# warmshao/ChatTTSPlus

Measured on AMD Instinct MI355X. Metric: decode tokens/s, higher is better.
Workload: dtype f32

## Files before the change

chatttsplus_amd/csrc/gpt_engine.hip:

```cpp
#include <fcntl.h>
#include <stdarg.h>
#include <stdio.h>
#include <stdlib.h>
#include <string.h>
#include <sys/file.h>
#include <sys/stat.h>
#include <unistd.h>

#include <cmath>
#include <map>
#include <mutex>
#include <string>
#include <atomic>
#include <thread>
#include <vector>

#include "../../include/ctts_hip.h"
#include "kernels.h"
#include "persist.h"
#include "roctx_range.h"

static thread_local char g_err[512] = "";
void ctts_set_error(const char* fmt, ...) {
    va_list ap;
// ... 1360 lines not shown
        CTTS_HIP_CHECK(hipMemcpyAsync(h->x_pre, emb + (size_t)r0 * h->H, (size_t)n * h->H * 4, hipMemcpyDeviceToDevice, s));
        if (run_layers(h, h->x_pre, h->meta_pre + r0, h->rope_pre + (size_t)r0 * 64, n, DecodePath{1, 0}, nullptr, s)) return 1;
        sr.cum[0] = 0;
        for (int b = 0; b < B; ++b) {
            const long s0 = (long)b * T + T - n_targets[b], s1 = (long)b * T + T;
            const long lo = s0 > r0 ? s0 : r0, hi = s1 < r0 + n ? s1 : r0 + n;
            const int cnt = hi > lo ? (int)(hi - lo) : 0;
            sr.first[b] = cnt ? (int)(lo - r0) : 0;
            sr.j0[b] = cnt ? (int)(lo - s0) : 0;
            sr.cum[b + 1] = sr.cum[b] + cnt;
        }
        for (int g0 = 0; g0 < sr.cum[B]; g0 += SCORE_ROWS) {
            const int m = sr.cum[B] - g0 < SCORE_ROWS ? sr.cum[B] - g0 : SCORE_ROWS;
            if (launch_score_gather(h->x_pre, h->score_x, h->score_oidx, g0, m, sr, s)) return 1;
            GemmArgs a = {};
            a.R = m; a.eps = 1e-6f; a.W = h->whead; a.n_row_tiles = (NV + 15) / 16; a.K = h->H; a.x = h->score_x; a.lnw = h->lnf;
            a.logits = h->score_logits; a.n_valid = NV;
            if (launch_gemm(h->cfg.dtype, nbg, PRO_NORM, EPI_LOGITS, a, (m + 16 * nbg - 1) / (16 * nbg), s)) return 1;
            if (launch_score_reduce(h->score_logits, h->score_oidx, targets, logprob, argmax, m, h->V, NV, s)) return 1;
        }
    }
    return 0;
}

static int run_decode_step(ctts_gpt* h, DecodePath path, hipStream_t s);
static inline DecodePath pick_decode_path(const ctts_gpt* h, int longest);

extern "C" int ctts_gpt_set_logprob_out(ctts_gpt* h, float* lp_raw, float* lp_sampled, void* stream) {
    if (!h || h->B == 0) { ctts_set_error("set_logprob_out: no generate state (call ctts_gpt_begin first)"); return 1; }
    if (h->text_mode) { ctts_set_error("set_logprob_out: the refine-text pass (infer_text) returns no log-probs; code mode only"); return 1; }
    if (h->sampled) { ctts_set_error("set_logprob_out: called after the first ctts_gpt_sample / ctts_gpt_decode of this call; set the buffers right after ctts_gpt_begin"); return 1; }
    float* const p[2] = {lp_raw, lp_sampled};
    static_assert(offsetof(SamplerDyn, lp_sampled) == offsetof(SamplerDyn, lp_raw) + sizeof(float*), "the two destinations are copied as one pair");
    CTTS_HIP_CHECK(hipMemcpyAsync((char*)h->dyn + offsetof(SamplerDyn, lp_raw), p, sizeof(p), hipMemcpyHostToDevice, (hipStream_t)stream));
    return 0;
}

extern "C" int ctts_gpt_sample(ctts_gpt* h, void* stream) {
    if (!h || h->B == 0) { ctts_set_error("sample: call begin first"); return 1; }
    CTTS_RANGE("ctts_gpt_sample");
    h->sampled = true;
    if (h->batch_inv) {
        if (ensure_persist_images(h)) return 1;
        return run_decode_step(h, pick_decode_path(h, 0), (hipStream_t)stream);
    }
    return run_sample_phase(h, plain_form(h), (hipStream_t)stream);
}

extern "C" int ctts_gpt_restart(ctts_gpt* h, void* stream) {
    if (!h || h->B == 0) { ctts_set_error("restart: call begin first"); return 1; }
    if (h->B != h->B0) { ctts_set_error("restart: rows were compacted away (a regenerate restarts the whole batch at step 0, gpt.py:496-525)"); return 1; }
    if (h->admitted) { ctts_set_error("restart: rows of this batch were handed to other utterances (ctts_gpt_admit); re-admit the utterance with attempt + 1 instead"); return 1; }
    hipStream_t s = (hipStream_t)stream;
    CTTS_HIP_CHECK(hipMemcpyAsync(h->x_dec, h->x_last, (size_t)h->B * h->H * 4, hipMemcpyDeviceToDevice, s));
    if (h->batch_inv) CTTS_HIP_CHECK(hipMemcpyAsync(h->rope_dec, h->rope_dec0, (size_t)h->B * 64 * 4, hipMemcpyDeviceToDevice, s));
    return reset_state(h, true, s);
}

static int advance_rows(ctts_gpt* h, int n_steps) {
    int longest = 1;
    for (int r = 0; r < h->B; ++r) {
        int c = h->row_ctx[r] + n_steps;
        if (c > h->row_cap[r]) c = h->row_cap[r];
        h->row_ctx[r] = c;
        if (c > longest) longest = c;
    }
    return longest;
}

static inline int decode_persist(const ctts_gpt* h, int B, int L) {
    const int rows = tuning(h).persist_rows;
    if (!(rows > 0 && h->pimg != nullptr && B <= rows && B <= PL_MAXR)) return 0;
    if (h->lora_rows && h->lora_mlp) return 0;
    if (h->lora_rows && !(h->persist_lora && h->persist_sched == 3 && h->lora_Af != nullptr && h->H == PL_H)) return 0;
    int cap = PL_ATT_BLOCKS / (PL_NH * B);
    cap = cap > PL_SMAX ? PL_SMAX : (cap < 1 ? 1 : cap);
    if (h->persist_splits > 0) cap = h->persist_splits < cap ? h->persist_splits : cap;
    if (B > PL_MAXR_ONE) {
        if (h->persist_sched != 3) return 0;
        return (L > (h->persist_max_keys > 0 ? h->persist_max_keys : h->persist_pair_keys - 128 * (B - PL_MAXR_ONE - 1))) ? 0 : 1;
    }
    if (L > (h->persist_max_keys > 0 ? h->persist_max_keys : 1400 * cap)) return 0;
    const int share = h->persist_share_keys > 0 ? h->persist_share_keys : PL_SHARE_KEYS;
    if (L <= share + 128) return 1;
    const int want = (L + share - 1) / share;
    return want > cap ? cap : want;
}

static inline DecodePath pick_decode_path(const ctts_gpt* h, int longest) { return {decode_splits(h, h->B, longest), decode_persist(h, h->B, longest)}; }

struct PersistTurn {
    std::mutex mu;
    hipEvent_t ev = nullptr;
    hipStream_t last = nullptr;
    bool pending = false;
};
static PersistTurn* persist_turn() {
    static std::mutex mu;
    static std::map<int, PersistTurn*> turns;
    int dev = 0;
    if (hipGetDevice(&dev) != hipSuccess) return nullptr;
    std::lock_guard<std::mutex> lk(mu);
    auto it = turns.find(dev);
    if (it != turns.end()) return it->second;
    PersistTurn* t = new PersistTurn();
    if (hipEventCreateWithFlags(&t->ev, hipEventDisableTiming) != hipSuccess) { delete t; return nullptr; }
    turns[dev] = t;
    return t;
}
struct PersistTurnGuard {
    PersistTurn* t = nullptr;
    hipStream_t s = nullptr;
    int rc = 0;
    PersistTurnGuard(bool persistent, hipStream_t stream) : s(stream) {
        if (!persistent) return;
        t = persist_turn();
        if (!t) return;
        t->mu.lock();
        if (t->pending && t->last != s && hipStreamWaitEvent(s, t->ev, 0) != hipSuccess) rc = 1;
    }
    ~PersistTurnGuard() {
        if (!t) return;
        if (hipEventRecord(t->ev, s) == hipSuccess) { t->last = s; t->pending = true; }
        t->mu.unlock();
    }
};

static int run_decode_step(ctts_gpt* h, DecodePath path, hipStream_t s) {
    StreamForm form = {};
    if (run_layers(h, h->x_dec, h->meta_dec, h->rope_dec, h->B, path, h->st, s, &form)) return 1;
    return run_sample_phase(h, form, s);
}

static int graph_span(const ctts_gpt* h, DecodePath path, int left) {
    return (path.persist && h->graph_steps_persist > h->graph_steps && left >= h->graph_steps_persist) ? h->graph_steps_persist : h->graph_steps;
}

static int ensure_graph(ctts_gpt* h, DecodePath path, int n_steps) {
    char sig[160];
    snprintf(sig, sizeof(sig), "%d|%d|%p|%d|%d|%d|%d|%d", h->B, h->text_mode, (void*)h->kv, path.splits, h->lora_rows + 2 * h->lora_mlp, h->opt_gen, path.persist, n_steps);
    std::string key(sig);
    if (h->lora_rows) key.append((const char*)h->lora_row_slots, (size_t)h->B);
    if (h->graph_gen != h->opt_gen || h->graphs.size() >= 96) {
        if (!h->graphs.empty()) {
            CTTS_HIP_CHECK(hipDeviceSynchronize());
            for (auto& kv : h->graphs) { (void)hipGraphExecDestroy(kv.second.exec); (void)hipGraphDestroy(kv.second.graph); }
            h->graphs.clear(); h->gexec = nullptr;
        }
        h->graph_gen = h->opt_gen;
    }
    auto it = h->graphs.find(key);
    if (it != h->graphs.end()) { h->gexec = it->second.exec; return 0; }
    ctts_gpt::GraphEntry ge = {nullptr, nullptr};
    CTTS_HIP_CHECK(hipStreamBeginCapture(h->cap_stream, hipStreamCaptureModeThreadLocal));
    int rc = 0;
    for (int i = 0; i < n_steps && !rc; ++i) rc = run_decode_step(h, path, h->cap_stream);
    hipError_t e = hipStreamEndCapture(h->cap_stream, &ge.graph);
    if (rc) { if (ge.graph) (void)hipGraphDestroy(ge.graph); return 1; }
    if (e != hipSuccess) { ctts_set_error("hipStreamEndCapture: %s", hipGetErrorString(e)); return 1; }
    e = hipGraphInstantiate(&ge.exec, ge.graph, nullptr, nullptr, 0);
    if (e != hipSuccess) { (void)hipGraphDestroy(ge.graph); ctts_set_error("hipGraphInstantiate: %s", hipGetErrorString(e)); return 1; }
    h->graphs[key] = ge;
    h->gexec = ge.exec;
    return 0;
}

static void plan_decode(ctts_gpt* h, int n_steps) {
// ... 311 lines not shown
```

chatttsplus_amd/csrc/persist.h:

```cpp
#pragma once
#include "common.h"

#define PL_GEMV_BLOCKS 192
#define PL_ATT_BLOCKS 64
#define PL_BLOCKS (PL_GEMV_BLOCKS + PL_ATT_BLOCKS)
#ifndef PL_EW_ONE_ROW
#define PL_EW_ONE_ROW 4
#endif
#define PL_EDGE_WAVES(R) ((R) == 1 ? PL_EW_ONE_ROW : 4)
#define PL_THREADS(R) ((8 + PL_EDGE_WAVES(R)) * 64)
#define PL_THREADS_MAX 768
#define PL_H 768
#define PL_I 3072
#define PL_NH 12
#define PL_MAXR_ONE 5
#define PL_MAXR 8
#define PL_SHARE_KEYS 384
#define PL_QKV_BYTES (12 * 768 * 4)
#define PL_O_BYTES (4 * 768 * 4)
#define PL_GU_BYTES (32 * 768 * 4)
#define PL_D_BYTES (4 * 3072 * 4)
#define PL_BLOCK_BYTES (PL_QKV_BYTES + PL_O_BYTES + PL_GU_BYTES + PL_D_BYTES)
#define PL_LAYER_BYTES ((size_t)PL_GEMV_BLOCKS * PL_BLOCK_BYTES)
#define PL_G_QKV (PL_MAXR * PL_NH * 192)
#define PL_G_ATT (PL_MAXR * PL_H)
#define PL_G_X1 (PL_MAXR * PL_H)
#define PL_G_ACT (PL_MAXR * PL_I)
#define PL_G_X (PL_MAXR * PL_H)
#define PL_SMAX 5
#define PL_G_PART (PL_ATT_BLOCKS * 66)
#define PL_HEAD_ROWS 14
#define PL_HEAD_FRAGS (7 * 2 * 3 * 64)
#define PL_G_U (PL_MAXR * 64)
#define PL_G_TOTAL (PL_G_QKV + PL_G_ATT + PL_G_X1 + PL_G_ACT + PL_G_X + PL_G_PART + PL_G_U)

struct PersistArgs {
    const char* w;
    const char* hw;
    int heads;
    float* logits;
    int n_valid;
    const float* lnf;
    const SamplerDyn* dyn;
    const RowState* rows;
    int half_w;
    int n_layers;
    float* x;
    const RowMeta* meta;
    const float* rope_rows;
    void* kv;
    size_t kv_per;
    int Lmax;
    unsigned long long* g_qkv;
    unsigned long long* g_att;
    unsigned long long* g_x1;
    unsigned long long* g_act;
    unsigned long long* g_x;
    unsigned long long* g_part;
    int S;
    unsigned* epoch;
    int* error;
    const int* done;
    unsigned long long* ts;
    float eps;
    int sched;
    int pace;
    int delay_act, delay_x, nap_qkv;
    int delay_att, delay;
    int nap;
    int fault;
    int poll;
    int lora;
    int delay_u;
    unsigned long long lslots;
    const float* la_qkv;
    const float* la;
    const float* lb;
    const float* lscale;
    size_t la_qkv_stride, la_stride;
    unsigned long long* g_u;
};

int launch_persist_layer(int R, const PersistArgs& a, hipStream_t s);
int launch_persist_repack_heads(int half_w, const void* whead, int n_tiles, void* dst, hipStream_t s);
int launch_persist_repack(int half_w, const void* qkv, const void* o, const void* gu, const void* d, void* dst, hipStream_t s);
int persist_configure();
```

chatttsplus_amd/csrc/persist_layer.hip:

```cpp
#include "kernels.h"
#include "persist.h"

typedef unsigned long long u64;

#ifndef PL_LB
#define PL_LB PL_THREADS_MAX
#endif
#define PL_SPIN_LIMIT (1u << 18)

typedef __attribute__((address_space(3))) int pl_lds_int;
#define PL_ABORT_GET(p_) __hip_atomic_load((pl_lds_int*)(p_), __ATOMIC_RELAXED, __HIP_MEMORY_SCOPE_WORKGROUP)
#define PL_ABORT_SET(p_) __hip_atomic_store((pl_lds_int*)(p_), 1, __ATOMIC_RELAXED, __HIP_MEMORY_SCOPE_WORKGROUP)
__device__ inline void store_granule(u64* g, unsigned tag, float v) {
    __hip_atomic_store(g, ((u64)tag << 32) | (u64)__builtin_bit_cast(unsigned, v), __ATOMIC_RELAXED, __HIP_MEMORY_SCOPE_AGENT);
}

template <int N, typename OffFn>
__device__ inline bool sweep(const u64* base, unsigned lane_elem, OffFn off, unsigned tag, float (&v)[N], int* err, int code, int* abort_s, int nap = 1) {
    const u64* p = base + lane_elem;
    asm volatile("" : "+v"(p));
#pragma unroll 1
    for (unsigned spins = 0;; ++spins) {
        bool ok = true;
#pragma unroll
// ... 66 lines not shown
    const __amdgpu_buffer_rsrc_t rsrc = __builtin_amdgcn_make_buffer_rsrc((void*)base, 0, (int)(total * 16u), 0x00020000);
    const unsigned voff = f0 * 16u;
#pragma unroll 1
    for (unsigned spins = 0;; ++spins) {
        bool ok = true;
#pragma unroll
        for (int k = 0; k < N; ++k) {
            const pl_u32x4 x = __builtin_amdgcn_raw_buffer_load_b128(rsrc, (int)voff, (int)(k * stride * 16u), (int)(16u | 0x80000000u));
            v[k] = x;
            if (TAIL && k == N - 1) ok = ok && ((x[3] - x[0] - x[1] - x[2] == tag) || (f0 + k * stride >= total));
            else ok = ok && (x[3] - x[0] - x[1] - x[2] == tag);
        }
        if (__all(ok)) return true;
        bool giveup = spins >= PL_SPIN_LIMIT || PL_ABORT_GET(abort_s) != 0;
        if (!giveup && (spins & 1023u) == 1023u) giveup = __hip_atomic_load(err, __ATOMIC_RELAXED, __HIP_MEMORY_SCOPE_AGENT) != 0;
        if (giveup) {
            if ((threadIdx.x & 63) == 0) { atomicCAS(err, 0, code); PL_ABORT_SET(abort_s); }
            return false;
        }
        for (int z = 0; z < nap; ++z) __builtin_amdgcn_s_sleep(2);
    }
}
template <int K0, int N, int NE, int TOT>
__device__ __forceinline__ void act16_chunk(const void* g_act, int e, unsigned tag, __attribute__((address_space(3))) float* xs, int* err, int* abort_s, int nap) {
    pl_u32x4 v[N];
    constexpr bool TAIL = (NE * (K0 + N) > TOT);
    const bool got = sweep16<N, TAIL>(g_act, (unsigned)TOT, (unsigned)(e + NE * K0), (unsigned)NE, tag, v, err, 5, abort_s, nap);
    (void)got;
    int ee = e;
    asm volatile("" : "+v"(ee));
#pragma unroll
    for (int k = 0; k < N; ++k) {
        const int f = ee + NE * (K0 + k);
        if (!(TAIL && k == N - 1) || f < TOT) {
            const int P = f / PL_A16_SLOTS, s = f - PL_A16_SLOTS * P;
            __attribute__((address_space(3))) float* const d = xs + 16 * P + 3 * s;
            const unsigned w0 = v[k][0], w1 = v[k][1], w2 = v[k][2];
            d[0] = __builtin_bit_cast(float, w0);
            if (s < 5) { d[1] = __builtin_bit_cast(float, w1); d[2] = __builtin_bit_cast(float, w2); }
        }
    }
}

template <typename OffFn>
__device__ inline void watch_sentinels(const u64* base, OffFn off, int n, unsigned tag, int lane, int* abort_s) {
    const u64* p0 = base + ((lane < n) ? off(lane) : 0);
    const u64* p1 = base + ((lane + 64 < n) ? off(lane + 64) : 0);
    asm volatile("" : "+v"(p0), "+v"(p1));
#pragma unroll 1
    for (unsigned spins = 0; spins < 8192u; ++spins) {
        bool ok = true;
        if (lane < n) ok = (unsigned)(__hip_atomic_load(p0, __ATOMIC_RELAXED, __HIP_MEMORY_SCOPE_AGENT) >> 32) == tag;
        if (lane + 64 < n) ok = ok && ((unsigned)(__hip_atomic_load(p1, __ATOMIC_RELAXED, __HIP_MEMORY_SCOPE_AGENT) >> 32) == tag);
        if (__all(ok) || PL_ABORT_GET(abort_s) != 0) return;
        __builtin_amdgcn_s_sleep(2);
    }
}

template <bool ON> __device__ inline int pl_opq(int idx) {
    if constexpr (ON) asm volatile("" : "+v"(idx));
    return idx;
}
__device__ inline float dot4(const f32x4 w, const f32x4 x, float acc) {
    return fmaf(w[3], x[3], fmaf(w[2], x[2], fmaf(w[1], x[1], fmaf(w[0], x[0], acc))));
}
__device__ inline float dot4(const half4 w, const f32x4 x, float acc) {
    return fmaf((float)w[3], x[3], fmaf((float)w[2], x[2], fmaf((float)w[1], x[1], fmaf((float)w[0], x[0], acc))));
}
template <typename WT> struct PlW;
template <> struct PlW<float> { typedef f32x4 frag; };
template <> struct PlW<half_t> { typedef half4 frag; };
template <typename WT> struct PlKV;
template <> struct PlKV<float> {
    f32x4 a, b;
    __device__ inline void load(const float* p) { a = *(const f32x4*)p; b = *(const f32x4*)(p + 4); }
    __device__ inline float at(int j) const { return j < 4 ? a[j & 3] : b[j & 3]; }
};
template <> struct PlKV<half_t> {
    half8 h;
    __device__ inline void load(const half_t* p) { h = *(const half8*)p; }
    __device__ inline float at(int j) const { return (float)h[j]; }
};
__device__ inline float pl_exp_diff(float m, float mn) { return (m == -INFINITY) ? 0.f : expf(m - mn); }

constexpr int pl_pow2(int n) { return n <= 1 ? 1 : n <= 2 ? 2 : n <= 4 ? 4 : n <= 8 ? 8 : 16; }
template <int CTRL, int C> __device__ inline void pl_rs_step(float* v, bool f) {
    if constexpr (C > 1) {
#pragma unroll
        for (int i = 0; i < C / 2; ++i) {
            const float keep = f ? v[i + C / 2] : v[i];
            const float give = f ? v[i] : v[i + C / 2];
            v[i] = keep + dpp_f<CTRL>(give);
        }
    } else v[0] += dpp_f<CTRL>(v[0]);
}
#define PL_FRONT_BYTES 4096
#ifndef PL_TAIL_ALL
#define PL_TAIL_ALL 1
#endif
#ifndef PL_TAIL_IT
#define PL_TAIL_IT 4
#endif
#define PL_RED_FLOATS (8 * 32 * 4)
template <int P> __device__ inline void pl_reduce_store(float (&v)[P], float* red, int wave, int lane, int base = 0) {
    static_assert(P == 1 || P == 2 || P == 4 || P == 8 || P == 16, "pad to a power of two");
    constexpr int C1 = P > 1 ? P / 2 : 1, C2 = P > 2 ? P / 4 : 1, C3 = P > 4 ? P / 8 : 1;
    const bool f0 = ((lane ^ (lane >> 2)) & 1) != 0, f1 = (((lane >> 1) ^ (lane >> 2)) & 1) != 0, f2 = (((lane >> 2) ^ (lane >> 3)) & 1) != 0, f3 = ((lane >> 3) & 1) != 0;
    pl_rs_step<DPP_XOR1, P>(v, f0);
    pl_rs_step<DPP_XOR2, C1>(v, f1);
    pl_rs_step<DPP_HALF_MIRROR, C2>(v, f2);
    pl_rs_step<DPP_MIRROR, C3>(v, f3);
    int idx = 0;
    bool writer = true;
    if (P > 1) idx += f0 ? P / 2 : 0; else writer = writer && !f0;
    if (C1 > 1) idx += f1 ? C1 / 2 : 0; else writer = writer && !f1;
    if (C2 > 1) idx += f2 ? C2 / 2 : 0; else writer = writer && !f2;
    if (C3 > 1) idx += f3 ? C3 / 2 : 0; else writer = writer && !f3;
    if (writer) red[(wave * 32 + base + idx) * 4 + (lane >> 4)] = v[0];
}
__device__ inline float pl_red(const float* red, int wave, int n) {
    const f32x4 p = *(const f32x4*)(red + (wave * 32 + n) * 4);
    return (p[0] + p[1]) + (p[2] + p[3]);
}
#define PL_PV(N_) float pv[pl_pow2(N_)]; _Pragma("unroll") for (int n_ = 0; n_ < pl_pow2(N_); ++n_) pv[n_] = 0.f

__device__ inline int pl_slot(unsigned long long slots, int r) { return (int)(signed char)(unsigned char)(slots >> (8 * r)); }
template <typename WT> struct PlLoraRegs {
    f32x4 qa_[3], qb_[3], oa_[3], ob_;
    template <typename Q> __device__ inline f32x4& qa(Q&, int j) { return qa_[j]; }
    template <typename Q> __device__ inline f32x4& qb(Q&, int j) { return qb_[j]; }
    template <typename O> __device__ inline f32x4& oa(O&, int j) { return oa_[j]; }
    template <typename Q> __device__ inline f32x4& ob(Q&) { return ob_; }
};
template <> struct PlLoraRegs<float> {
    __device__ inline f32x4& qa(f32x4 (&q_w)[2][3], int j) { return q_w[0][j]; }
    __device__ inline f32x4& qb(f32x4 (&q_w)[2][3], int j) { return q_w[1][j]; }
    __device__ inline f32x4& oa(f32x4 (&o_w)[3], int j) { return o_w[j]; }
    __device__ inline f32x4& ob(f32x4 (&q_w)[2][3]) { return q_w[0][0]; }
};
template <int N>
__device__ inline bool sweep_masked(const u64* base, unsigned lane_elem, bool valid, unsigned tag, float (&v)[N], int* err, int code, int* abort_s, int nap) {
    const u64* p = base + (valid ? lane_elem : 0u);
    asm volatile("" : "+v"(p));
#pragma unroll
    for (int k = 0; k < N; ++k) v[k] = 0.f;
    if (!__any(valid)) return true;
#pragma unroll 1
    for (unsigned spins = 0;; ++spins) {
        bool ok = true;
        if (valid) {
#pragma unroll
            for (int k = 0; k < N; ++k) {
                const u64 x = __hip_atomic_load(p + k, __ATOMIC_RELAXED, __HIP_MEMORY_SCOPE_AGENT);
                v[k] = __builtin_bit_cast(float, (unsigned)x);
                ok = ok && ((unsigned)(x >> 32) == tag);
            }
        }
        if (__all(ok)) return true;
        bool giveup = spins >= PL_SPIN_LIMIT || PL_ABORT_GET(abort_s) != 0;
        if (!giveup && (spins & 1023u) == 1023u) giveup = __hip_atomic_load(err, __ATOMIC_RELAXED, __HIP_MEMORY_SCOPE_AGENT) != 0;
        if (giveup) {
            if ((threadIdx.x & 63) == 0) { atomicCAS(err, 0, code); PL_ABORT_SET(abort_s); }
            return false;
        }
        for (int z = 0; z < nap; ++z) __builtin_amdgcn_s_sleep(2);
    }
}

template <int R, int SCHED, typename WT, bool LORA = false>
__global__ __launch_bounds__(PL_LB) void persist_layer_kernel(const PersistArgs a) {
    static_assert(!LORA || SCHED == 3, "per-utterance adapters: the paced schedule only");
    typedef typename PlW<WT>::frag wfrag;
    constexpr bool A16 = PL_ACT16 != 0 && R <= PL_A16_MAXR;
    constexpr int EW = PL_EDGE_WAVES(R), NE = 64 * EW, GX = 768 / NE;
    constexpr size_t BLOCK_BYTES = (size_t)PL_BLOCK_BYTES / 4 * sizeof(WT), LAYER_BYTES = PL_LAYER_BYTES / 4 * sizeof(WT);
    extern __shared__ __attribute__((aligned(16))) char smem[];
    int* const abort_s = (int*)smem;
    float* const att_s = (float*)(abort_s + 4);
    float* const xs = (float*)(smem + PL_FRONT_BYTES);
    float* const red = xs + R * PL_I;
    float* const ssq = red + PL_RED_FLOATS;
    float* const xres = ssq + 4 * R;
    float* const lbs = xres + 4 * R;
    const int tid = threadIdx.x, lane = tid & 63;
    const int wave = __builtin_amdgcn_readfirstlane(tid >> 6);
    const int b = blockIdx.x;
    const int done_v = vload_flag(a.done), err_v = vload_flag(a.error), ep_v = vload_flag((const int*)a.epoch);
    const int NL = a.n_layers;
    unsigned long long t_mark[10];
#define PL_MARK(i) do { if (a.ts != nullptr) t_mark[i] = wall_clock64(); } while (0)
    PL_MARK(0);
    if (tid == 0) { abort_s[0] = 0; abort_s[1] = 0; }

    if (b < PL_GEMV_BLOCKS) {
        const char* wb = a.w + (size_t)b * BLOCK_BYTES;
        if (wave < 8) {
            const size_t oq = (size_t)wave * (2 * 3 * 64) + lane;
            const size_t oo = (size_t)PL_QKV_BYTES / 16 + (size_t)wave * (3 * 64) + lane;
            const size_t og = (size_t)(PL_QKV_BYTES + PL_O_BYTES) / 16 + (size_t)wave * (4 * 3 * 64) + lane;
            const size_t od = (size_t)(PL_QKV_BYTES + PL_O_BYTES + PL_GU_BYTES) / 16 + (size_t)wave * (6 * 64) + lane;
            wfrag q_w[2][3], o_w[3], g_w[4][3], d_w[6];
#define PL_LOAD_Q(base_) do { if (wave < 6) { _Pragma("unroll") for (int row = 0; row < 2; ++row) _Pragma("unroll") for (int j = 0; j < 3; ++j) \
                q_w[row][j] = __builtin_nontemporal_load((const wfrag*)(base_) + oq + (row * 3 + j) * 64); } } while (0)
#define PL_LOAD_O(base_) do { if (wave < 4) { _Pragma("unroll") for (int j = 0; j < 3; ++j) o_w[j] = __builtin_nontemporal_load((const wfrag*)(base_) + oo + j * 64); } } while (0)
#define PL_LOAD_G(base_) do { _Pragma("unroll") for (int s = 0; s < 4; ++s) _Pragma("unroll") for (int j = 0; j < 3; ++j) \
                g_w[s][j] = __builtin_nontemporal_load((const wfrag*)(base_) + og + (s * 3 + j) * 64); } while (0)
#define PL_LOAD_D(base_) do { _Pragma("unroll") for (int j = 0; j < 6; ++j) d_w[j] = __builtin_nontemporal_load((const wfrag*)(base_) + od + j * 64); } while (0)
            PL_LOAD_Q(wb);
            if (SCHED == 1) PL_LOAD_O(wb);
            PlLoraRegs<WT> lr;
            const unsigned tag0c = (unsigned)ep_v * 32u;
            const int lw = 2 * b + (wave - 6), ll = (wave - 6) * 64 + lane;
            const int lq_r = lw / 48, lq_tk = lw - 48 * lq_r;
            const int lq_sl = (LORA && wave >= 6 && lq_r < R) ? pl_slot(a.lslots, lq_r) : -1;
            const int lo_r = lw >> 4, lo_k = lw & 15;
            const int lo_sl = (LORA && wave >= 6 && lo_r < R) ? pl_slot(a.lslots, lo_r) : -1;
            constexpr int LQM = (192 * R + 127) / 128, LOM = (64 * R + 127) / 128;
#define PL_LORA_REQ_QKV(l_) do { if (wave >= 6) { \
                if (lq_sl >= 0) { const f32x4* ap_ = (const f32x4*)(a.la_qkv + (size_t)(l_) * a.la_qkv_stride + (size_t)(lq_sl * 48 + lq_tk) * PL_H); \
                    _Pragma("unroll") for (int j = 0; j < 3; ++j) lr.qa(q_w, j) = ap_[64 * j + lane]; \
                    lq_scale = a.lscale[((l_) * 8 + lq_sl) * 4 + (lq_tk >> 4)]; } \
                int li_ = ll; asm volatile("" : "+v"(li_)); \
                _Pragma("unroll") for (int m = 0; m < LQM; ++m) { const int i_ = li_ + 128 * m; float v_ = 0.f; \
                    if (i_ < 192 * R) { const int r_ = i_ / 192, rem_ = i_ - 192 * r_, j_ = rem_ >> 4, k_ = rem_ & 15, sl_ = pl_slot(a.lslots, r_); \
                        if (sl_ >= 0) { const int pw_ = j_ >> 1, hf_ = j_ & 1, hh_ = b >> 4, jj_ = b & 15; \
                            const int t_ = pw_ < 4 ? (pw_ >> 1) : 2, d_ = pw_ < 4 ? 2 * jj_ + (pw_ & 1) + 32 * hf_ : 4 * jj_ + 2 * (pw_ - 4) + hf_; \
                            v_ = a.lb[(size_t)(l_) * a.la_stride + (size_t)((sl_ * 4 + t_) * 16 + k_) * PL_H + hh_ * 64 + d_]; } } \
                    lr.qb(q_w, m >> 2)[m & 3] = v_; } } } while (0)
#define PL_LORA_REQ_O(l_) do { if (wave >= 6) { \
                if (lo_sl >= 0) { const f32x4* ap_ = (const f32x4*)(a.la + (size_t)(l_) * a.la_stride + (size_t)((lo_sl * 4 + 3) * 16 + lo_k) * PL_H); \
                    _Pragma("unroll") for (int j = 0; j < 3; ++j) lr.oa(o_w, j) = ap_[64 * j + lane]; \
                    lo_scale = a.lscale[((l_) * 8 + lo_sl) * 4 + 3]; } \
                int li_ = ll; asm volatile("" : "+v"(li_)); \
                _Pragma("unroll") for (int m = 0; m < LOM; ++m) { const int i_ = li_ + 128 * m; float v_ = 0.f; \
                    if (i_ < 64 * R) { const int r_ = i_ >> 6, ii_ = (i_ >> 4) & 3, k_ = i_ & 15, sl_ = pl_slot(a.lslots, r_); \
                        if (sl_ >= 0) v_ = a.lb[(size_t)(l_) * a.la_stride + (size_t)((sl_ * 4 + 3) * 16 + k_) * PL_H + 4 * b + ii_]; } \
                    lr.ob(q_w)[m] = v_; } } } while (0)
            float lq_scale = 0.f, lo_scale = 0.f;
            if constexpr (LORA) PL_LORA_REQ_QKV(0);
            __builtin_amdgcn_sched_barrier(0);
            if (__builtin_amdgcn_readfirstlane(done_v | err_v)) return;
            __syncthreads();
            if constexpr (SCHED == 3) {
                typedef __attribute__((address_space(3))) int lds_int;
                lds_int* const arrive = (lds_int*)(abort_s + 1);
                int phase = 0;
                const int pace = a.pace;
#define PL_PACE_BEGIN() const int tgt_ = EW * (++phase); bool ready_ = __hip_atomic_load(arrive, __ATOMIC_RELAXED, __HIP_MEMORY_SCOPE_WORKGROUP) >= tgt_
#define PL_PIECE(stmt_) do { stmt_; if (!ready_) { for (int z_ = 0; z_ < pace; ++z_) __builtin_amdgcn_s_sleep(2); ready_ = __hip_atomic_load(arrive, __ATOMIC_RELAXED, __HIP_MEMORY_SCOPE_WORKGROUP) >= tgt_; } } while (0)
#define PL_PACE_END() do { while (!ready_) { __builtin_amdgcn_s_sleep(1); ready_ = __hip_atomic_load(arrive, __ATOMIC_RELAXED, __HIP_MEMORY_SCOPE_WORKGROUP) >= tgt_; } asm volatile("" ::: "memory"); } while (0)
                for (int l = 0; l < NL; ++l) {
                    const char* const wn = wb + LAYER_BYTES;
                    const bool more = l + 1 < NL;
                    {
                        PL_PACE_BEGIN();
                        if (wave < 4) {
#pragma unroll
// ... 302 lines not shown
            const unsigned tag0 = (unsigned)ep_v * 32u;
            if (e < R) *(f32x4*)(xres + 4 * e) = xown;
            float ssp[R];
#pragma unroll
            for (int r = 0; r < R; ++r) ssp[r] = 0.f;
#pragma unroll
            for (int i = 0; i < XIT; ++i) {
                const int idx = e + NE * i;
                if (idx < R * 192) ((f32x4*)xs)[idx] = xv[i];
                const float d = xv[i][0] * xv[i][0] + xv[i][1] * xv[i][1] + xv[i][2] * xv[i][2] + xv[i][3] * xv[i][3];
#pragma unroll
                for (int r = 0; r < R; ++r) ssp[r] += (idx / 192 == r) ? d : 0.f;
            }
#pragma unroll
            for (int r = 0; r < R; ++r) {
                const float s = wave_sum(ssp[r]);
                if (lane == 0) ssq[ew * R + r] = s;
            }
            __syncthreads();
            PL_MARK(1);
            const size_t kv_per = a.kv_per;
            for (int l = 0; l < NL; ++l) {
                const unsigned tag = tag0 + (unsigned)l;
                const bool last = l + 1 == NL;
                if (l > 0) {
                    for (int z = 0; z < a.delay_x; ++z) __builtin_amdgcn_s_sleep(2);
                    if (EW == 2 && (a.poll & 1)) watch_sentinels(a.g_x, [ew](int i) { return (R - 1) * PL_H + 4 * (16 * (2 * (i >> 4) + ew) + (i & 15)) + 3; }, 96, tag - 1u, lane, abort_s);
                    float v[GX * R];
                    const bool got = PL_SWEEP(GX * R, a.g_x, PL_G_X, (unsigned)e, [](int k) { return (k / GX) * PL_H + NE * (k % GX); }, tag - 1u, v, 1);
                    (void)got;
#pragma unroll
                    for (int r = 0; r < R; ++r) ssp[r] = 0.f;
#pragma unroll
                    for (int k = 0; k < GX * R; ++k) {
                        xs[(k / GX) * PL_H + NE * (k % GX) + e] = v[k];
                        ssp[k / GX] += v[k] * v[k];
                    }
#pragma unroll
                    for (int r = 0; r < R; ++r) {
                        const float s = wave_sum(ssp[r]);
                        if (lane == 0) ssq[ew * R + r] = s;
                    }
                }
                if (last) PL_MARK(2);
                PL_B1();
                float lda = 0.f, ldb = 0.f;
                float uq[LORA ? 16 : 1];
                const int slA = (LORA && doA) ? pl_slot(a.lslots, rA) : -1;
                if constexpr (LORA) {
                    for (int z = 0; z < a.delay_u; ++z) __builtin_amdgcn_s_sleep(2);
                    const bool got = sweep_masked<16>(a.g_u, (unsigned)(rA * 64 + (pwA < 4 ? (pwA >> 1) : 2) * 16), slA >= 0, tag, uq, a.error, 9, abort_s, a.nap);
                    (void)got;
                }
                __syncthreads();
                if constexpr (LORA) {
                    if (slA >= 0) {
                        const float* const bq = lbs + rA * 192 + 2 * pwA * 16;
#pragma unroll
                        for (int k = 0; k < 16; ++k) { lda = fmaf(bq[k], uq[k], lda); ldb = fmaf(bq[16 + k], uq[k], ldb); }
                    }
                }
                if (doA) {
                    const float rs = 1.0f / sqrtf((EW == 2 ? ssq[rA] + ssq[R + rA] : (ssq[rA] + ssq[R + rA]) + (ssq[2 * R + rA] + ssq[3 * R + rA])) / (float)PL_H + a.eps);
                    const float va = pl_red(red, pwA, rA) * rs + lda, vb = pl_red(red, pwA, R + rA) * rs + ldb;
                    float ya = va, yb = vb;
                    int which, dA, dB;
                    if (pwA < 4) {
                        which = pwA >> 1; dA = 2 * jj + (pwA & 1); dB = dA + 32;
                        ya = __fadd_rn(__fmul_rn(va, cA), __fmul_rn(-vb, sA));
                        yb = __fadd_rn(__fmul_rn(vb, cA), __fmul_rn(va, sA));
                    } else {
                        which = 2; dA = 4 * jj + 2 * (pwA - 4); dB = dA + 1;
                    }
                    u64* const gq = a.g_qkv + (size_t)pl_opq<(R > PL_MAXR_ONE)>((rA * PL_NH + hh) * 192 + which * 64);
                    store_granule(gq + dA, tag, ya);
                    store_granule(gq + dB, tag, yb);
                    if (which >= 1) {
                        WT* c = (WT*)a.kv + (size_t)l * 2 * kv_per + (which == 2 ? kv_per : 0) + (((size_t)mA.seq * PL_NH + hh) * a.Lmax + mA.slot) * CTTS_HEAD_DIM;
                        c[dA] = (WT)ya; c[dB] = (WT)yb;
                    }
                }
                if (last) PL_MARK(3);
                for (int z = 0; z < a.delay_att; ++z) __builtin_amdgcn_s_sleep(2);
                {
                    if (EW == 2 && (a.poll & 1)) watch_sentinels(a.g_att, [ew](int i) { return (i / 6) * PL_H + 64 * (2 * (i % 6) + ew) + 63; }, 6 * R, tag, lane, abort_s);
                    float v[GX * R];
                    const bool got = PL_SWEEP(GX * R, a.g_att, PL_G_ATT, (unsigned)e, [](int k) { return (k / GX) * PL_H + NE * (k % GX); }, tag, v, 3);
                    (void)got;
#pragma unroll
                    for (int k = 0; k < GX * R; ++k) xs[(k / GX) * PL_H + NE * (k % GX) + e] = v[k];
                }
                if (last) PL_MARK(4);
                PL_B1();
                float ldo = 0.f;
                float uo[LORA ? 16 : 1];
                const int slO = (LORA && e < 4 * R) ? pl_slot(a.lslots, e >> 2) : -1;
                if constexpr (LORA) {
                    for (int z = 0; z < a.delay_u; ++z) __builtin_amdgcn_s_sleep(2);
                    const bool got = sweep_masked<16>(a.g_u, (unsigned)((e >> 2) * 64 + 48), slO >= 0, tag, uo, a.error, 10, abort_s, a.nap);
                    (void)got;
                }
                __syncthreads();
                if constexpr (LORA) {
                    if (slO >= 0) {
                        const float* const bo = lbs + 192 * R + (e >> 2) * 64 + (e & 3) * 16;
#pragma unroll
                        for (int k = 0; k < 16; ++k) ldo = fmaf(bo[k], uo[k], ldo);
                    }
                }
                if (e < 4 * R) {
                    const int i = e & 3, r = e >> 2;
                    const float x1 = xres[4 * r + i] + (pl_red(red, i, r) + ldo);
                    xres[4 * r + i] = x1;
                    if (!(a.fault > 0 && b == 5 && l + 1 == a.fault))
                        store_granule(a.g_x1 + (size_t)pl_opq<(R > PL_MAXR_ONE)>(r * PL_H + 4 * b + i), tag, x1);
                }
                if (last) PL_MARK(5);
                for (int z = 0; z < a.delay; ++z) __builtin_amdgcn_s_sleep(2);
                {
                    if (EW == 2 && (a.poll & 1)) watch_sentinels(a.g_x1, [ew](int i) { return (R - 1) * PL_H + 4 * (16 * (2 * (i >> 4) + ew) + (i & 15)) + 3; }, 96, tag, lane, abort_s);
                    float v[GX * R];
                    const bool got = PL_SWEEP(GX * R, a.g_x1, PL_G_X1, (unsigned)e, [](int k) { return (k / GX) * PL_H + NE * (k % GX); }, tag, v, 4);
                    (void)got;
#pragma unroll
                    for (int r = 0; r < R; ++r) ssp[r] = 0.f;
#pragma unroll
                    for (int k = 0; k < GX * R; ++k) {
                        xs[(k / GX) * PL_H + NE * (k % GX) + e] = v[k];
                        ssp[k / GX] += v[k] * v[k];
                    }
#pragma unroll
                    for (int r = 0; r < R; ++r) {
                        const float s = wave_sum(ssp[r]);
                        if (lane == 0) ssq[ew * R + r] = s;
                    }
                }
                if (last) PL_MARK(6);
                PL_B1();
                __syncthreads();
                if constexpr (A16) {
                    float av = 0.f;
                    const int pi = e & 15, r = e >> 4;
                    if (e < 16 * R) {
                        const int w = pi >> 1, p = pi & 1;
                        const float rs = 1.0f / sqrtf((EW == 2 ? ssq[r] + ssq[R + r] : (ssq[r] + ssq[R + r]) + (ssq[2 * R + r] + ssq[3 * R + r])) / (float)PL_H + a.eps);
                        const float gv = pl_red(red, w, 16 * p + r) * rs, uv = pl_red(red, w, 16 * p + R + r) * rs;
                        av = (gv / (1.0f + expf(-gv))) * uv;
                    }
                    const float a1 = __shfl_down(av, 1), a2 = __shfl_down(av, 2);
                    if (e < 16 * R && pi % 3 == 0)
                        store_granule16(a.g_act, PL_GEMV_BLOCKS * PL_A16_SLOTS * R, (unsigned)pl_opq<(R > PL_MAXR_ONE)>((r * PL_GEMV_BLOCKS + b) * PL_A16_SLOTS + pi / 3), tag,
                                        av, (pi + 1 < 16) ? a1 : 0.f, (pi + 2 < 16) ? a2 : 0.f);
                } else if (e < 16 * R) {
                    const int pi = e & 15, r = e >> 4, w = pi >> 1, p = pi & 1;
                    const float rs = 1.0f / sqrtf((EW == 2 ? ssq[r] + ssq[R + r] : (ssq[r] + ssq[R + r]) + (ssq[2 * R + r] + ssq[3 * R + r])) / (float)PL_H + a.eps);
                    const float gv = pl_red(red, w, 16 * p + r) * rs, uv = pl_red(red, w, 16 * p + R + r) * rs;
                    store_granule(a.g_act + (size_t)pl_opq<(R > PL_MAXR_ONE)>(r * PL_I + 16 * b + pi), tag, (gv / (1.0f + expf(-gv))) * uv);
                }
                if (last) PL_MARK(7);
                for (int z = 0; z < a.delay_act; ++z) __builtin_amdgcn_s_sleep(2);
                if constexpr (A16) {
                    constexpr int TOT = PL_GEMV_BLOCKS * PL_A16_SLOTS * R, NK = (TOT + NE - 1) / NE;
                    constexpr int NC = (NK + PL_A16_CHUNK - 1) / PL_A16_CHUNK, CH = (NK + NC - 1) / NC;
                    act16_chunk<0, (NK < CH ? NK : CH), NE, TOT>(a.g_act, e, tag, (__attribute__((address_space(3))) float*)xs, a.error, abort_s, a.nap);
                    if constexpr (NC > 1) act16_chunk<CH, (NK - CH < CH ? NK - CH : CH), NE, TOT>(a.g_act, e, tag, (__attribute__((address_space(3))) float*)xs, a.error, abort_s, a.nap);
                    if constexpr (NC > 2) act16_chunk<2 * CH, (NK - 2 * CH < CH ? NK - 2 * CH : CH), NE, TOT>(a.g_act, e, tag, (__attribute__((address_space(3))) float*)xs, a.error, abort_s, a.nap);
                    if constexpr (NC > 3) act16_chunk<3 * CH, (NK - 3 * CH < CH ? NK - 3 * CH : CH), NE, TOT>(a.g_act, e, tag, (__attribute__((address_space(3))) float*)xs, a.error, abort_s, a.nap);
// ... 230 lines not shown
            if constexpr (NT > 0) {
#pragma unroll
                for (int t = 0; t < NT; ++t) {
                    if (any_ok[PRE + t]) {
                        const float pe = (sc[PRE + t] == -INFINITY) ? 0.f : expf(sc[PRE + t] - mrun);
                        lrun += pe;
#pragma unroll
                        for (int g = 0; g < 8; ++g) {
                            float vt;
                            if constexpr (sizeof(WT) == 4) vt = *(const __attribute__((address_space(3))) float*)(tl + t * TB + 2048 + g * 256 + lane * 4);
                            else vt = (float)*(const __attribute__((address_space(3))) half_t*)(tl + t * TB + 1024 + g * 128 + lane * 2);
                            oa[g & 3] = fmaf(readlane_f(pe, 8 * g), vt, oa[g & 3]);
                        }
                    }
                }
            }
            constexpr int UNS = 4, STEP = 8 * NWI;
            for (int wb0 = kv0 + 8 * (iw + NWI * PT); wb0 < kv1; wb0 += STEP * UNS) {
                PlKV<WT> ks_[UNS];
                typename KvElem<WT>::reg vs_[UNS][8];
                bool live_[UNS];
#pragma unroll
                for (int u = 0; u < UNS; ++u) {
                    const int p0 = wb0 + STEP * u;
                    live_[u] = p0 + grp < kv1;
                    ks_[u].load(kb + (size_t)(live_[u] ? p0 + grp : m.kv_start) * CTTS_HEAD_DIM);
#pragma unroll
                    for (int g = 0; g < 8; ++g) vs_[u][g] = KvElem<WT>::load(vb + (size_t)min(p0 + g, kv1 - 1) * CTTS_HEAD_DIM);
                }
#pragma unroll
                for (int u = 0; u < UNS; ++u) {
                    if (wb0 + STEP * u >= kv1) break;
                    const bool live = live_[u];
                    float dot = q0[0] * ks_[u].at(0) + q0[1] * ks_[u].at(1) + q0[2] * ks_[u].at(2) + q0[3] * ks_[u].at(3) + q1[0] * ks_[u].at(4) + q1[1] * ks_[u].at(5) + q1[2] * ks_[u].at(6) + q1[3] * ks_[u].at(7);
                    dot += dpp_f<DPP_XOR1>(dot);
                    dot += dpp_f<DPP_XOR2>(dot);
                    dot += dpp_f<DPP_HALF_MIRROR>(dot);
                    const float mn = wave_max(fmaxf(mrun, live ? dot : -INFINITY));
                    const float scl = pl_exp_diff(mrun, mn);
                    const float pe = live ? expf(dot - mn) : 0.f;
                    lrun = lrun * scl + pe;
#pragma unroll
                    for (int i = 0; i < 4; ++i) oa[i] *= scl;
#pragma unroll
                    for (int g = 0; g < 8; ++g) oa[g & 3] = fmaf(readlane_f(pe, 8 * g), KvElem<WT>::f(vs_[u][g]), oa[g & 3]);
                    mrun = mn;
                }
            }
            PL_AMARK(5);
            const float lw = wave_sum(lrun) * 0.125f;
            mo[wave * 64 + lane] = (oa[0] + oa[1]) + (oa[2] + oa[3]);
            if (lane == 0) { mm[wave] = mrun; ml[wave] = lw; }
            PL_AMARK(6);
            __syncthreads();
            if (l + 1 < NL) { PL_DMA_KV(l + 1); PL_LOAD_KV(l + 1); }
            __builtin_amdgcn_sched_barrier(0);
        }
    } else if (wave == 8 || (PAIR && wave == 9)) {
        if (__builtin_amdgcn_readfirstlane(done_v | err_v)) return;
        const unsigned tag0 = (unsigned)ep_v * 32u;
        __syncthreads();
        for (int l = 0; l < NL; ++l) {
            const unsigned tag = tag0 + (unsigned)l;
            float v[3];
            const bool got = sweep<3>(a.g_qkv, (unsigned)(rh * 192 + lane), [](int k) { return 64 * k; }, tag, v, a.error, 2, abort_s, a.nap_qkv);
            (void)got;
            qs[lane] = v[0] * 0.125f;
            ks[lane] = v[1];
            vs[lane] = v[2];
            if (l + 1 == NL && wave == 8) PL_MARK(1);
            __syncthreads();
            const float dnew = wave_sum(qs[lane] * ks[lane]);
            __syncthreads();
            if (a.ts != nullptr && l + 1 == NL && lane == 0 && wave == 8) a.ts[(size_t)b * 10 + 7] = wall_clock64();
            const float mmv = mm[NWI * isub + (lane & (NWI - 1))], mlv = ml[NWI * isub + (lane & (NWI - 1))];
            const float mj = (lane < NWI) ? mmv : ((lane == NWI && sp == 0) ? dnew : -INFINITY);
            const float lj = (lane < NWI) ? mlv : ((lane == NWI) ? 1.f : 0.f);
            float M = wave_max(mj);
            const float sj = pl_exp_diff(mj, M);
            float L = wave_sum(sj * lj);
            float O = readlane_f(sj, NWI) * vs[lane];
#pragma unroll
            for (int w = 0; w < NWI; ++w) O = fmaf(readlane_f(sj, w), mo[(NWI * isub + w) * 64 + lane], O);
            if (S > 1 && sp != 0) {
                u64* const gp = a.g_part + (size_t)(rh * S + sp) * 66;
                store_granule(gp + 2 + lane, tag, O);
                if (lane == 0) store_granule(gp, tag, M);
                if (lane == 1) store_granule(gp + 1, tag, L);
            } else {
                if (S > 1) {
                    const u64* p = a.g_part + (size_t)(rh * S) * 66;
                    asm volatile("" : "+v"(p));
                    float po[4], pm[4], pl[4];
#pragma unroll 1
                    for (unsigned spins = 0;; ++spins) {
                        bool okk = true;
#pragma unroll
                        for (int t = 0; t < 4; ++t) {
                            if (t + 1 < S) {
                                const u64 xo = __hip_atomic_load(p + (t + 1) * 66 + 2 + lane, __ATOMIC_RELAXED, __HIP_MEMORY_SCOPE_AGENT);
                                const u64 xm = __hip_atomic_load(p + (t + 1) * 66, __ATOMIC_RELAXED, __HIP_MEMORY_SCOPE_AGENT);
                                const u64 xl = __hip_atomic_load(p + (t + 1) * 66 + 1, __ATOMIC_RELAXED, __HIP_MEMORY_SCOPE_AGENT);
                                po[t] = __builtin_bit_cast(float, (unsigned)xo); pm[t] = __builtin_bit_cast(float, (unsigned)xm); pl[t] = __builtin_bit_cast(float, (unsigned)xl);
                                okk = okk && ((unsigned)(xo >> 32) == tag) && ((unsigned)(xm >> 32) == tag) && ((unsigned)(xl >> 32) == tag);
                            }
                        }
                        if (__all(okk)) break;
                        typedef __attribute__((address_space(3))) int lds_i;
                        bool giveup = spins >= PL_SPIN_LIMIT || __hip_atomic_load((lds_i*)abort_s, __ATOMIC_RELAXED, __HIP_MEMORY_SCOPE_WORKGROUP) != 0;
                        if (!giveup && (spins & 1023u) == 1023u) giveup = __hip_atomic_load(a.error, __ATOMIC_RELAXED, __HIP_MEMORY_SCOPE_AGENT) != 0;
                        if (giveup) { if (lane == 0) { atomicCAS(a.error, 0, 6); __hip_atomic_store((lds_i*)abort_s, 1, __ATOMIC_RELAXED, __HIP_MEMORY_SCOPE_WORKGROUP); } break; }
                        __builtin_amdgcn_s_sleep(2);
                    }
#pragma unroll
                    for (int t = 0; t < 4; ++t) {
                        if (t + 1 < S) {
                            const float mn = fmaxf(M, pm[t]);
                            const float s1 = pl_exp_diff(M, mn), s2 = pl_exp_diff(pm[t], mn);
                            L = L * s1 + pl[t] * s2;
                            O = O * s1 + po[t] * s2;
                            M = mn;
                        }
                    }
                }
                store_granule(a.g_att + (size_t)r * PL_H + hh * CTTS_HEAD_DIM + lane, tag, O / L);
            }
            if (l + 1 == NL && wave == 8) PL_MARK(2);
        }
        if (a.ts != nullptr && lane == 0 && wave == 8) {
            a.ts[(size_t)b * 10 + 0] = t_mark[0]; a.ts[(size_t)b * 10 + 1] = t_mark[1]; a.ts[(size_t)b * 10 + 2] = t_mark[2];
        }
    } else {
        if (__builtin_amdgcn_readfirstlane(done_v | err_v)) return;
        __syncthreads();
        for (int l = 0; l < NL; ++l) {
            __syncthreads();
            __syncthreads();
        }
    }
}

template <typename WT>
__global__ __launch_bounds__(256) void persist_repack_kernel(const typename PlW<WT>::frag* qkv, const typename PlW<WT>::frag* o, const typename PlW<WT>::frag* gu,
                                                             const typename PlW<WT>::frag* d, typename PlW<WT>::frag* dst) {
    const int idx = blockIdx.x * 256 + threadIdx.x;
    if (idx >= PL_GEMV_BLOCKS * (PL_BLOCK_BYTES / 16)) return;
    const int g = idx / (PL_BLOCK_BYTES / 16), oo = idx % (PL_BLOCK_BYTES / 16);
    const typename PlW<WT>::frag* src;
    int row_tile, i, k4, ktiles;
    if (oo < PL_QKV_BYTES / 16) {
        const int pw = oo / 384, rem = oo % 384, row = rem / 192, j = (rem % 192) / 64, ln = rem % 64;
        const int hh = g >> 4, jj = g & 15;
        int which, dd;
        if (pw < 4) { which = pw >> 1; dd = 2 * jj + (pw & 1) + 32 * row; }
        else { which = 2; dd = 4 * jj + 2 * (pw - 4) + row; }
        row_tile = which * 48 + hh * 4 + (dd & 31) / 8;
        i = (dd & 7) + (dd >= 32 ? 8 : 0);
        k4 = 64 * j + ln; ktiles = 48; src = qkv;
    } else if (oo < (PL_QKV_BYTES + PL_O_BYTES) / 16) {
        const int o2 = oo - PL_QKV_BYTES / 16, w = o2 / 192, rem = o2 % 192, j = rem / 64, ln = rem % 64;
        const int row = 4 * g + w;
        row_tile = row >> 4; i = row & 15; k4 = 64 * j + ln; ktiles = 48; src = o;
    } else if (oo < (PL_QKV_BYTES + PL_O_BYTES + PL_GU_BYTES) / 16) {
        const int o2 = oo - (PL_QKV_BYTES + PL_O_BYTES) / 16, w = o2 / 768, rem = o2 % 768, s = rem / 192, j = (rem % 192) / 64, ln = rem % 64;
        const int dim = 16 * g + 2 * w + (s >> 1), isup = s & 1;
        row_tile = dim >> 3; i = (dim & 7) + 8 * isup;
        k4 = 64 * j + ln; ktiles = 48; src = gu;
    } else {
        const int o2 = oo - (PL_QKV_BYTES + PL_O_BYTES + PL_GU_BYTES) / 16, w = o2 / 384, rem = o2 % 384, j = rem / 64, ln = rem % 64;
        const int row = 4 * g + (w >> 1);
        row_tile = row >> 4; i = row & 15; k4 = 384 * (w & 1) + 64 * j + ln; ktiles = 192; src = d;
    }
    if constexpr (sizeof(WT) == 4) dst[idx] = src[((size_t)row_tile * ktiles + (k4 >> 2)) * 64 + i + 16 * (k4 & 3)];
    else dst[idx] = src[(((size_t)row_tile * (ktiles / 2) + (k4 >> 3)) * 64 + i + 16 * ((k4 >> 1) & 3)) * 2 + (k4 & 1)];
}

template <typename WT>
__global__ __launch_bounds__(256) void persist_repack_heads_kernel(const typename PlW<WT>::frag* whead, int n_tiles, typename PlW<WT>::frag* dst) {
    const int idx = blockIdx.x * 256 + threadIdx.x;
    if (idx >= PL_GEMV_BLOCKS * PL_HEAD_FRAGS) return;
    const int g = idx / PL_HEAD_FRAGS, o2 = idx % PL_HEAD_FRAGS, w = o2 / 384, rem = o2 % 384, row = rem / 192, j = (rem % 192) / 64, ln = rem % 64;
    const int hrow = PL_HEAD_ROWS * g + 2 * w + row, row_tile = hrow >> 4, i = hrow & 15, k4 = 64 * j + ln;
    typename PlW<WT>::frag v = {};
    if (row_tile < n_tiles) {
        if constexpr (sizeof(WT) == 4) v = whead[((size_t)row_tile * 48 + (k4 >> 2)) * 64 + i + 16 * (k4 & 3)];
        else v = whead[(((size_t)row_tile * 24 + (k4 >> 3)) * 64 + i + 16 * ((k4 >> 1) & 3)) * 2 + (k4 & 1)];
    }
    dst[idx] = v;
}
int launch_persist_repack_heads(int half_w, const void* whead, int n_tiles, void* dst, hipStream_t s) {
    const int n = PL_GEMV_BLOCKS * PL_HEAD_FRAGS;
    if (half_w) hipLaunchKernelGGL(persist_repack_heads_kernel<half_t>, dim3((n + 255) / 256), dim3(256), 0, s, (const half4*)whead, n_tiles, (half4*)dst);
    else hipLaunchKernelGGL(persist_repack_heads_kernel<float>, dim3((n + 255) / 256), dim3(256), 0, s, (const f32x4*)whead, n_tiles, (f32x4*)dst);
    CTTS_HIP_CHECK(hipGetLastError());
    return 0;
}

int launch_persist_repack(int half_w, const void* qkv, const void* o, const void* gu, const void* d, void* dst, hipStream_t s) {
    const int n = PL_GEMV_BLOCKS * (PL_BLOCK_BYTES / 16);
    if (half_w) hipLaunchKernelGGL(persist_repack_kernel<half_t>, dim3((n + 255) / 256), dim3(256), 0, s, (const half4*)qkv, (const half4*)o, (const half4*)gu, (const half4*)d, (half4*)dst);
    else hipLaunchKernelGGL(persist_repack_kernel<float>, dim3((n + 255) / 256), dim3(256), 0, s, (const f32x4*)qkv, (const f32x4*)o, (const f32x4*)gu, (const f32x4*)d, (f32x4*)dst);
    CTTS_HIP_CHECK(hipGetLastError());
    return 0;
}

static size_t persist_lds_bytes(int R) {
    const size_t gemv = (size_t)(R * PL_I + PL_RED_FLOATS + 4 * R + 4 * R + 256 * R) * 4, tail = (R > PL_MAXR_ONE || PL_TAIL_ALL) ? (size_t)8 * PL_TAIL_IT * 4096 : 0;
// ... 66 lines not shown
```

Measured before the change: 3900.

## Move split-key attention merge from share-0 block into consumer GEMV gather

Attention blocks for every key share now write their partial (O, M, L) as one 16-byte granule per lane. Previously share 0 spin-waited on the other shares, merged them and then published the result. The consuming GEMV waves now gather all shares with 128-bit buffer loads and fold the online-softmax partials themselves, writing the merged values straight into LDS. This removes one cross-block wait-and-publish hop in the split-attention path. In exchange the consumers do redundant merge work and more global loads, and the partial buffer layout changes.

```diff
diff --git a/chatttsplus_amd/csrc/gpt_engine.hip b/chatttsplus_amd/csrc/gpt_engine.hip
--- a/chatttsplus_amd/csrc/gpt_engine.hip
+++ b/chatttsplus_amd/csrc/gpt_engine.hip
@@ -1466,7 +1466,7 @@
     }
     if (L > (h->persist_max_keys > 0 ? h->persist_max_keys : 1400 * cap)) return 0;
     const int share = h->persist_share_keys > 0 ? h->persist_share_keys : PL_SHARE_KEYS;
-    if (L <= share + 128) return 1;
+    if (L <= share + PL_ONE_SHARE_TAIL) return 1;
     const int want = (L + share - 1) / share;
     return want > cap ? cap : want;
 }
diff --git a/chatttsplus_amd/csrc/persist.h b/chatttsplus_amd/csrc/persist.h
--- a/chatttsplus_amd/csrc/persist.h
+++ b/chatttsplus_amd/csrc/persist.h
@@ -16,6 +16,7 @@
 #define PL_MAXR_ONE 5
 #define PL_MAXR 8
 #define PL_SHARE_KEYS 384
+#define PL_ONE_SHARE_TAIL 128
 #define PL_QKV_BYTES (12 * 768 * 4)
 #define PL_O_BYTES (4 * 768 * 4)
 #define PL_GU_BYTES (32 * 768 * 4)
@@ -28,7 +29,8 @@
 #define PL_G_ACT (PL_MAXR * PL_I)
 #define PL_G_X (PL_MAXR * PL_H)
 #define PL_SMAX 5
-#define PL_G_PART (PL_ATT_BLOCKS * 66)
+#define PL_G_PART_GRANULES (PL_ATT_BLOCKS * 64)
+#define PL_G_PART (PL_G_PART_GRANULES * 2)
 #define PL_HEAD_ROWS 14
 #define PL_HEAD_FRAGS (7 * 2 * 3 * 64)
 #define PL_G_U (PL_MAXR * 64)
diff --git a/chatttsplus_amd/csrc/persist_layer.hip b/chatttsplus_amd/csrc/persist_layer.hip
--- a/chatttsplus_amd/csrc/persist_layer.hip
+++ b/chatttsplus_amd/csrc/persist_layer.hip
@@ -172,6 +172,65 @@
     __device__ inline float at(int j) const { return (float)h[j]; }
 };
 __device__ inline float pl_exp_diff(float m, float mn) { return (m == -INFINITY) ? 0.f : expf(m - mn); }
+
+template <int S>
+__device__ inline float pl_fold_shares(const pl_u32x4 (&p)[S]) {
+    unsigned w0 = p[0][0], w1 = p[0][1], w2 = p[0][2];
+    float O = __builtin_bit_cast(float, w0), M = __builtin_bit_cast(float, w1), L = __builtin_bit_cast(float, w2);
+#pragma unroll
+    for (int t = 1; t < S; ++t) {
+        w0 = p[t][0]; w1 = p[t][1]; w2 = p[t][2];
+        const float Ot = __builtin_bit_cast(float, w0), Mt = __builtin_bit_cast(float, w1), Lt = __builtin_bit_cast(float, w2);
+        const float mn = fmaxf(M, Mt);
+        const float s1 = pl_exp_diff(M, mn), s2 = pl_exp_diff(Mt, mn);
+        L = fmaf(L, s1, __fmul_rn(Lt, s2));
+        O = fmaf(O, s1, __fmul_rn(Ot, s2));
+        M = mn;
+    }
+    return O / L;
+}
+template <int R, int GX, int NE, int S, int C0, int CN>
+__device__ __forceinline__ void att_merge_chunk(const void* g_part, int ew, int lane, unsigned tag, __attribute__((address_space(3))) float* xs, int* err, int* abort_s, int nap) {
+    constexpr int HPC = NE / 64;
+    static_assert((((R - 1) * PL_NH + HPC * (GX - 1) + HPC - 1) * S + S) * 64 <= PL_G_PART_GRANULES, "g_part: more granules than the buffer holds");
+    const __amdgpu_buffer_rsrc_t rsrc = __builtin_amdgcn_make_buffer_rsrc((void*)g_part, 0, (int)(PL_G_PART_GRANULES * 16u), 0x00020000);
+    const unsigned voff = (unsigned)lane * 16u;
+    unsigned s0 = (unsigned)ew * (S * 1024u);
+    asm volatile("" : "+s"(s0));
+    pl_u32x4 v[CN][S];
+#pragma unroll 1
+    for (unsigned spins = 0;; ++spins) {
+        bool ok = true;
+#pragma unroll
+        for (int c = C0; c < C0 + CN; ++c)
+#pragma unroll
+            for (int t = 0; t < S; ++t) {
+                const pl_u32x4 x = __builtin_amdgcn_raw_buffer_load_b128(rsrc, (int)voff, (int)(s0 + (unsigned)((((c / GX) * PL_NH + HPC * (c % GX)) * S + t) * 1024)), (int)(16u | 0x80000000u));
+                v[c - C0][t] = x;
+                ok = ok && (x[3] - x[0] - x[1] - x[2] == tag);
+            }
+        if (__all(ok)) break;
+        bool giveup = spins >= PL_SPIN_LIMIT || PL_ABORT_GET(abort_s) != 0;
+        if (!giveup && (spins & 1023u) == 1023u) giveup = __hip_atomic_load(err, __ATOMIC_RELAXED, __HIP_MEMORY_SCOPE_AGENT) != 0;
+        if (giveup) {
+            if (lane == 0) { atomicCAS(err, 0, 3); PL_ABORT_SET(abort_s); }
+            break;
+        }
+        for (int z = 0; z < nap; ++z) __builtin_amdgcn_s_sleep(2);
+    }
+#pragma unroll
+    for (int c = C0; c < C0 + CN; ++c) xs[(c / GX) * PL_H + NE * (c % GX) + 64 * ew + lane] = pl_fold_shares<S>(v[c - C0]);
+}
+template <int R, int GX, int NE, int S, int MAXG>
+__device__ __forceinline__ void att_merge_gather(const void* g_part, int ew, int lane, unsigned tag, __attribute__((address_space(3))) float* xs, int* err, int* abort_s, int nap) {
+    constexpr int NC = GX * R, H = (NC + 1) / 2;
+    if constexpr (NC * S <= MAXG) att_merge_chunk<R, GX, NE, S, 0, NC>(g_part, ew, lane, tag, xs, err, abort_s, nap);
+    else {
+        static_assert(H * S <= MAXG, "key shares: more chunks");
+        att_merge_chunk<R, GX, NE, S, 0, H>(g_part, ew, lane, tag, xs, err, abort_s, nap);
+        att_merge_chunk<R, GX, NE, S, H, NC - H>(g_part, ew, lane, tag, xs, err, abort_s, nap);
+    }
+}
 
 constexpr int pl_pow2(int n) { return n <= 1 ? 1 : n <= 2 ? 2 : n <= 4 ? 4 : n <= 8 ? 8 : 16; }
 template <int CTRL, int C> __device__ inline void pl_rs_step(float* v, bool f) {
@@ -263,6 +322,7 @@
     typedef typename PlW<WT>::frag wfrag;
     constexpr bool A16 = PL_ACT16 != 0 && R <= PL_A16_MAXR;
     constexpr int EW = PL_EDGE_WAVES(R), NE = 64 * EW, GX = 768 / NE;
+    constexpr int SCAP = (PL_ATT_BLOCKS / (PL_NH * R) < PL_SMAX) ? (PL_ATT_BLOCKS / (PL_NH * R) < 1 ? 1 : PL_ATT_BLOCKS / (PL_NH * R)) : PL_SMAX;
     constexpr size_t BLOCK_BYTES = (size_t)PL_BLOCK_BYTES / 4 * sizeof(WT), LAYER_BYTES = PL_LAYER_BYTES / 4 * sizeof(WT);
     extern __shared__ __attribute__((aligned(16))) char smem[];
     int* const abort_s = (int*)smem;
@@ -731,7 +791,18 @@
                 }
                 if (last) PL_MARK(3);
                 for (int z = 0; z < a.delay_att; ++z) __builtin_amdgcn_s_sleep(2);
-                {
+                bool merged = false;
+                if constexpr (SCAP > 1) {
+                    __attribute__((address_space(3))) float* const xl = (__attribute__((address_space(3))) float*)xs;
+                    merged = a.S > 1;
+                    constexpr int MG = sizeof(WT) == 2 ? 12 : 16;
+                    if (a.S == 2) att_merge_gather<R, GX, NE, 2, MG>(a.g_part, ew, lane, tag, xl, a.error, abort_s, a.nap);
+                    if constexpr (SCAP >= 3) if (a.S == 3) att_merge_gather<R, GX, NE, 3, MG>(a.g_part, ew, lane, tag, xl, a.error, abort_s, a.nap);
+                    if constexpr (SCAP >= 4) if (a.S == 4) att_merge_gather<R, GX, NE, 4, MG>(a.g_part, ew, lane, tag, xl, a.error, abort_s, a.nap);
+                    if constexpr (SCAP >= 5) if (a.S == 5) att_merge_gather<R, GX, NE, 5, MG>(a.g_part, ew, lane, tag, xl, a.error, abort_s, a.nap);
+                    static_assert(SCAP <= 5, "key shares: more merge instantiations");
+                }
+                if (!merged) {
                     if (EW == 2 && (a.poll & 1)) watch_sentinels(a.g_att, [ew](int i) { return (i / 6) * PL_H + 64 * (2 * (i % 6) + ew) + 63; }, 6 * R, tag, lane, abort_s);
                     float v[GX * R];
                     const bool got = PL_SWEEP(GX * R, a.g_att, PL_G_ATT, (unsigned)e, [](int k) { return (k / GX) * PL_H + NE * (k % GX); }, tag, v, 3);
@@ -1128,47 +1199,9 @@
             float O = readlane_f(sj, NWI) * vs[lane];
 #pragma unroll
             for (int w = 0; w < NWI; ++w) O = fmaf(readlane_f(sj, w), mo[(NWI * isub + w) * 64 + lane], O);
-            if (S > 1 && sp != 0) {
-                u64* const gp = a.g_part + (size_t)(rh * S + sp) * 66;
-                store_granule(gp + 2 + lane, tag, O);
-                if (lane == 0) store_granule(gp, tag, M);
-                if (lane == 1) store_granule(gp + 1, tag, L);
+            if (S > 1) {
+                store_granule16(a.g_part, (unsigned)PL_G_PART_GRANULES, (unsigned)(item * 64 + lane), tag, O, M, L);
             } else {
-                if (S > 1) {
-                    const u64* p = a.g_part + (size_t)(rh * S) * 66;
-                    asm volatile("" : "+v"(p));
-                    float po[4], pm[4], pl[4];
-#pragma unroll 1
-                    for (unsigned spins = 0;; ++spins) {
-                        bool okk = true;
-#pragma unroll
-                        for (int t = 0; t < 4; ++t) {
-                            if (t + 1 < S) {
-                                const u64 xo = __hip_atomic_load(p + (t + 1) * 66 + 2 + lane, __ATOMIC_RELAXED, __HIP_MEMORY_SCOPE_AGENT);
-                                const u64 xm = __hip_atomic_load(p + (t + 1) * 66, __ATOMIC_RELAXED, __HIP_MEMORY_SCOPE_AGENT);
-                                const u64 xl = __hip_atomic_load(p + (t + 1) * 66 + 1, __ATOMIC_RELAXED, __HIP_MEMORY_SCOPE_AGENT);
-                                po[t] = __builtin_bit_cast(float, (unsigned)xo); pm[t] = __builtin_bit_cast(float, (unsigned)xm); pl[t] = __builtin_bit_cast(float, (unsigned)xl);
-                                okk = okk && ((unsigned)(xo >> 32) == tag) && ((unsigned)(xm >> 32) == tag) && ((unsigned)(xl >> 32) == tag);
-                            }
-                        }
-                        if (__all(okk)) break;
-                        typedef __attribute__((address_space(3))) int lds_i;
-                        bool giveup = spins >= PL_SPIN_LIMIT || __hip_atomic_load((lds_i*)abort_s, __ATOMIC_RELAXED, __HIP_MEMORY_SCOPE_WORKGROUP) != 0;
-                        if (!giveup && (spins & 1023u) == 1023u) giveup = __hip_atomic_load(a.error, __ATOMIC_RELAXED, __HIP_MEMORY_SCOPE_AGENT) != 0;
-                        if (giveup) { if (lane == 0) { atomicCAS(a.error, 0, 6); __hip_atomic_store((lds_i*)abort_s, 1, __ATOMIC_RELAXED, __HIP_MEMORY_SCOPE_WORKGROUP); } break; }
-                        __builtin_amdgcn_s_sleep(2);
-                    }
-#pragma unroll
-                    for (int t = 0; t < 4; ++t) {
-                        if (t + 1 < S) {
-                            const float mn = fmaxf(M, pm[t]);
-                            const float s1 = pl_exp_diff(M, mn), s2 = pl_exp_diff(pm[t], mn);
-                            L = L * s1 + pl[t] * s2;
-                            O = O * s1 + po[t] * s2;
-                            M = mn;
-                        }
-                    }
-                }
                 store_granule(a.g_att + (size_t)r * PL_H + hh * CTTS_HEAD_DIM + lane, tag, O / L);
             }
             if (l + 1 == NL && wave == 8) PL_MARK(2);
```

New measurement: 3868. Within noise of the previous version (-0.8%).
